# jzbontar/mc-cnn

Hardware: AMD Instinct MI355X
Metric: Mega-pixel-disparities/sec (cost-vol+CBCA+SGM) + end-to-end disp ms/pair (higher is better)
Workload: dtype f32; 1 GPU; KITTI 2012 fast, 370x1226 disp_max=228; H=370, W=1226, disp_max=228, feature_channels=64, params=kitti_fast, parallelism=one pair per GPU

## Files before the change

mc-cnn_amd/csrc/post.hip:

```cpp
#include "launchers.h"

#include <atomic>

namespace mc {


__global__ void __launch_bounds__(256) fill_nan_kernel(float *__restrict__ p, int64_t n)
{
	const float nanv = __builtin_nanf("");
	for (int64_t i = (int64_t)blockIdx.x * blockDim.x + threadIdx.x; i < n; i += (int64_t)gridDim.x * blockDim.x) p[i] = nanv;
}

__global__ void __launch_bounds__(256) scale_kernel(const float *__restrict__ in, float *__restrict__ out, int64_t n, float s)
{
	for (int64_t i = (int64_t)blockIdx.x * blockDim.x + threadIdx.x; i < n; i += (int64_t)gridDim.x * blockDim.x) out[i] = in[i] * s;
}
typedef float f4v_t __attribute__((ext_vector_type(4)));
__global__ void __launch_bounds__(256) scale4_kernel(const f4v_t *__restrict__ in, f4v_t *__restrict__ out, int64_t n4, float s)
{
	const int64_t i = (int64_t)blockIdx.x * 256 + threadIdx.x;
	if (i < n4) out[i] = in[i] * s;
}

template <bool NT>
__global__ void __launch_bounds__(256) transpose_kernel(const float *__restrict__ in, float *__restrict__ out, int64_t R,
                                                        int64_t Cn, int64_t ldin, int64_t ldout, float s)
{
	__shared__ float tile[64][65];
	const int64_t c0 = (int64_t)blockIdx.x * 64, r0 = (int64_t)blockIdx.y * 64;
	const int tx = threadIdx.x & 63, ty = threadIdx.x >> 6;
	for (int k = ty; k < 64; k += 4) {
		const int64_t r = r0 + k, c = c0 + tx;
		if (r < R && c < Cn) tile[k][tx] = NT ? __builtin_nontemporal_load(in + r * ldin + c) : in[r * ldin + c];
	}
	__syncthreads();
	for (int k = ty; k < 64; k += 4) {
		const int64_t c = c0 + k, r = r0 + tx;
		if (r < R && c < Cn) {
			if (NT) __builtin_nontemporal_store(tile[tx][k] * s, out + c * ldout + r);
			else out[c * ldout + r] = tile[tx][k] * s;
		}
	}
}

typedef float post_f4 __attribute__((ext_vector_type(4)));
template <bool NT, bool LOOP_R>
__global__ void __launch_bounds__(256) transpose4_kernel(const float *__restrict__ in, float *__restrict__ out, int64_t R,
                                                         int64_t Cn, int64_t ldin, int64_t ldout, float s)
{
	__shared__ float tile[64][65];
	const int lx = threadIdx.x & 15, ly = threadIdx.x >> 4;
	const int64_t fixed0 = (int64_t)blockIdx.x * 64;
	const int64_t nloop = LOOP_R ? R : Cn;
	for (int64_t t0 = 0; t0 < nloop; t0 += 64) {
		const int64_t c0 = LOOP_R ? fixed0 : t0, r0 = LOOP_R ? t0 : fixed0;
#pragma unroll
		for (int k = 0; k < 4; ++k) {
			const int row = ly + 16 * k;
			const int64_t r = r0 + row, c = c0 + 4 * lx;
			if (r < R && c < Cn) {
				const post_f4 *p = (const post_f4 *)(in + r * ldin + c);
				const post_f4 v = NT ? __builtin_nontemporal_load(p) : *p;
				tile[row][4 * lx + 0] = v.x; tile[row][4 * lx + 1] = v.y; tile[row][4 * lx + 2] = v.z; tile[row][4 * lx + 3] = v.w;
			}
		}
		__syncthreads();
#pragma unroll
		for (int k = 0; k < 4; ++k) {
			const int col = ly + 16 * k;
			const int64_t c = c0 + col, r = r0 + 4 * lx;
			if (c < Cn && r < R) {
				const post_f4 v = {tile[4 * lx + 0][col] * s, tile[4 * lx + 1][col] * s, tile[4 * lx + 2][col] * s, tile[4 * lx + 3][col] * s};
				post_f4 *q = (post_f4 *)(out + c * ldout + r);
				if (NT) __builtin_nontemporal_store(v, q);
				else *q = v;
			}
		}
		__syncthreads();
	}
}


int fill_nan(float *p, int64_t n, hipStream_t st)
{
	if (n <= 0) return 0;
	const unsigned blocks = cdiv(n, 256) < 4096u ? cdiv(n, 256) : 4096u;
	hipLaunchKernelGGL(fill_nan_kernel, dim3(blocks), dim3(256), 0, st, p, n);
	return check_launch("fill_nan");
}

int scale(const float *in, float *out, int64_t n, float s, hipStream_t st)
{
	if (n <= 0) return 0;
	if (n % 4 == 0 && (uintptr_t)in % 16 == 0 && (uintptr_t)out % 16 == 0 && n / 4 / 256 < 0x7fffffff) {
		hipLaunchKernelGGL(scale4_kernel, dim3(cdiv(n / 4, 256)), dim3(256), 0, st, (const f4v_t *)in, (f4v_t *)out, n / 4, s);
		return check_launch("scale");
	}
	const unsigned blocks = cdiv(n, 256) < 4096u ? cdiv(n, 256) : 4096u;
	hipLaunchKernelGGL(scale_kernel, dim3(blocks), dim3(256), 0, st, in, out, n, s);
	return check_launch("scale");
}

int transpose(const float *in, float *out, int64_t R, int64_t Cn, int64_t ldin, int64_t ldout, float s, hipStream_t st, int nt)
{
	const bool use_nt = nt >= 0 ? nt != 0 : R * Cn * 4 > ((int64_t)768 << 20);
	const bool aligned16 = Cn % 4 == 0 && ldin % 4 == 0 && ldout % 4 == 0 && (uintptr_t)in % 16 == 0 && (uintptr_t)out % 16 == 0;
	if (R % 4 == 0 && aligned16) {
		if (R <= Cn) {
			if (use_nt) hipLaunchKernelGGL((transpose4_kernel<true, true>), dim3(cdiv(Cn, 64)), dim3(256), 0, st, in, out, R, Cn, ldin, ldout, s);
			else hipLaunchKernelGGL((transpose4_kernel<false, true>), dim3(cdiv(Cn, 64)), dim3(256), 0, st, in, out, R, Cn, ldin, ldout, s);
		} else {
			if (use_nt) hipLaunchKernelGGL((transpose4_kernel<true, false>), dim3(cdiv(R, 64)), dim3(256), 0, st, in, out, R, Cn, ldin, ldout, s);
			else hipLaunchKernelGGL((transpose4_kernel<false, false>), dim3(cdiv(R, 64)), dim3(256), 0, st, in, out, R, Cn, ldin, ldout, s);
		}
		return check_launch("transpose");
	}
	if (use_nt) hipLaunchKernelGGL(transpose_kernel<true>, dim3(cdiv(Cn, 64), cdiv(R, 64)), dim3(256), 0, st, in, out, R, Cn, ldin, ldout, s);
	else hipLaunchKernelGGL(transpose_kernel<false>, dim3(cdiv(Cn, 64), cdiv(R, 64)), dim3(256), 0, st, in, out, R, Cn, ldin, ldout, s);
	return check_launch("transpose");
}

__global__ void __launch_bounds__(256) fix_border_kernel(float *__restrict__ vol, int64_t rows, int W, int n, int direction)
{
	const int64_t id = (int64_t)blockIdx.x * blockDim.x + threadIdx.x;
	if (id >= rows * n) return;
	const int i = (int)(id % n) + 1;
	const int64_t r = id / n;
	const int dst = direction < 0 ? W - i : i - 1;
	const int src = direction < 0 ? W - (n + 1) : n;
	vol[r * W + dst] = vol[r * W + src];
}

int fix_border(float *vol, int D, int H, int W, int n, int direction, hipStream_t st)
{
	if (n <= 0) return 0;
	const int64_t rows = (int64_t)D * H;
	hipLaunchKernelGGL(fix_border_kernel, dim3(cdiv(rows * n, 256)), dim3(256), 0, st, vol, rows, W, n, direction);
	return check_launch("fix_border");
}

__global__ void __launch_bounds__(256) argmin_dhw_kernel(const float *__restrict__ vol, float *__restrict__ out, int D, int64_t HW,
                                                         int base1)
{
	const int64_t p = (int64_t)blockIdx.x * blockDim.x + threadIdx.x;
	if (p >= HW) return;
	int argmin = 0;
	float mn = __builtin_inff();
	for (int i = 0; i < D; ++i) {
		const float val = __builtin_nontemporal_load(vol + i * HW + p);
		if (val < mn) {
			mn = val;
			argmin = i;
		}
	}
	out[p] = (float)(argmin + base1);
}

__global__ void __launch_bounds__(256) argmin_dhw4_kernel(const float *__restrict__ vol, float *__restrict__ out, int D, int64_t HW,
                                                          int base1)
{
	const int64_t p = ((int64_t)blockIdx.x * blockDim.x + threadIdx.x) * 4;
	if (p >= HW) return;
	int a0 = 0, a1 = 0, a2 = 0, a3 = 0;
	float m0 = __builtin_inff(), m1 = m0, m2 = m0, m3 = m0;
	for (int i = 0; i < D; ++i) {
		const post_f4 v = __builtin_nontemporal_load((const post_f4 *)(vol + i * HW + p));
		if (v.x < m0) { m0 = v.x; a0 = i; }
		if (v.y < m1) { m1 = v.y; a1 = i; }
		if (v.z < m2) { m2 = v.z; a2 = i; }
		if (v.w < m3) { m3 = v.w; a3 = i; }
	}
	*(post_f4 *)(out + p) = post_f4{(float)(a0 + base1), (float)(a1 + base1), (float)(a2 + base1), (float)(a3 + base1)};
}

int argmin_dhw(const float *vol, float *out, int D, int H, int W, int base1, hipStream_t st)
{
	const int64_t HW = (int64_t)H * W;
	if (HW % 4 == 0 && (uintptr_t)vol % 16 == 0 && (uintptr_t)out % 16 == 0)
		hipLaunchKernelGGL(argmin_dhw4_kernel, dim3(cdiv(HW / 4, 256)), dim3(256), 0, st, vol, out, D, HW, base1);
	else
		hipLaunchKernelGGL(argmin_dhw_kernel, dim3(cdiv(HW, 256)), dim3(256), 0, st, vol, out, D, HW, base1);
	return check_launch("argmin_dhw");
}

__global__ void __launch_bounds__(256) outlier_rows_kernel(const float *__restrict__ d0, const float *__restrict__ d1,
                                                           float *__restrict__ outlier, int W, int disp_max)
{
	extern __shared__ unsigned char mark[];
	const int y = blockIdx.x;
	const int64_t row = (int64_t)y * W;
	for (int x = threadIdx.x; x < W; x += 256) mark[x] = 0;
	__syncthreads();
	for (int xp = threadIdx.x; xp < W; xp += 256) {
		const float v = d1[row + xp];
		if (v > -2.0f && v < (float)disp_max + 2.0f) {
			const int base = (int)floorf(v);
#pragma unroll
			for (int k = -2; k <= 3; ++k) {
				const int d = base + k;
				if (d >= 0 && d < disp_max && xp + d < W && (double)fabsf((float)d - v) < 1.1) mark[xp + d] = 1;
			}
		}
	}
	__syncthreads();
	for (int x = threadIdx.x; x < W; x += 256) {
		const int64_t id = row + x;
		const int d0i = (int)d0[id];
		float res;
		if (x - d0i < 0) res = 1;
		else if ((double)fabsf(d0[id] - d1[id - d0i]) < 1.1) res = 0;
		else res = mark[x] ? 2.0f : 1.0f;
		outlier[id] = res;
	}
}

struct LdsRaised {
	std::atomic<int> cus[64] = {};
	int raise(const void *kernel, int bytes, const char *who, int *ncu = nullptr)
	{
		int dev = 0;
		hipError_t e = hipGetDevice(&dev);
		if (e == hipSuccess && (dev < 0 || dev >= 64)) e = hipErrorInvalidDevice;
		if (e != hipSuccess) {
			set_error("%s: hipGetDevice: %s (device %d)", who, hipGetErrorString(e), dev);
			return (int)e;
		}
		int n = cus[dev].load(std::memory_order_acquire);
		if (!n) {
			e = hipFuncSetAttribute(kernel, hipFuncAttributeMaxDynamicSharedMemorySize, bytes);
			if (e == hipSuccess) e = hipDeviceGetAttribute(&n, hipDeviceAttributeMultiprocessorCount, dev);
			if (e != hipSuccess || n <= 0) {
				set_error("%s: %d bytes of dynamic LDS on device %d: %s", who, bytes, dev, hipGetErrorString(e));
				return e != hipSuccess ? (int)e : MC_EINVAL;
			}
			cus[dev].store(n, std::memory_order_release);
		}
		if (ncu) *ncu = n;
		return 0;
	}
};

int outlier_detection(const float *d0, const float *d1, float *outlier, int H, int W, int disp_max, hipStream_t st)
{
	MC_REQUIRE(W <= 160 * 1024, "outlier_detection: a row of %d pixels needs more than the 160 KiB of LDS its marks live in", W);
	if (W > 64 * 1024) {
		static LdsRaised raised;
		const int rc = raised.raise((const void *)outlier_rows_kernel, 160 * 1024, "outlier_detection");
		if (rc) return rc;
	}
	hipLaunchKernelGGL(outlier_rows_kernel, dim3(H), dim3(256), (size_t)W, st, d0, d1, outlier, W, disp_max);
	return check_launch("outlier_detection");
}

__global__ void __launch_bounds__(256) interp_occ_rows_kernel(const float *__restrict__ d0, const float *__restrict__ outlier,
                                                              float *__restrict__ out, int W, unsigned *__restrict__ mask, int size)
{
	__shared__ int carry[256];
	__shared__ int first_valid;
	const int y = blockIdx.x, t = threadIdx.x;
	const int64_t row = (int64_t)y * W;
	if (mask) {
		const int wa = (int)((row + 31) >> 5), wb = (int)((row + W + 31) >> 5);
		for (int w0 = wa; w0 < wb; w0 += 8) {
			const int p = w0 * 32 + t;
			const uint64_t bal = __ballot(p < size && outlier[p] == 2);
			const int w = w0 + (t >> 5);
			if ((t & 31) == 0 && w < wb) mask[w] = (unsigned)(bal >> (t & 32));
		}
	}
	const int seg = (W + 255) / 256;
	const int xa = t * seg, xb = min(W, xa + seg);
	if (t == 0) first_valid = W;
	int last = -1;
	for (int x = xa; x < xb; ++x)
		if (outlier[row + x] == 0) last = x;
	carry[t] = last;
	__syncthreads();
	if (last >= 0) {
		int f = -1;
		for (int x = xa; x < xb; ++x)
			if (outlier[row + x] == 0) { f = x; break; }
		atomicMin(&first_valid, f);
	}
	for (int off = 1; off < 256; off <<= 1) {
		const int o = t >= off ? carry[t - off] : -1;
		__syncthreads();
		carry[t] = max(carry[t], o);
		__syncthreads();
	}
	int lv = t > 0 ? carry[t - 1] : -1;
	const int fv = first_valid;
	for (int x = xa; x < xb; ++x) {
		const int64_t id = row + x;
		const float o = outlier[id];
		if (o == 0) lv = x;
		float r = d0[id];
		if (o == 1) {
			if (lv >= 0) r = d0[row + lv];
			else if (fv < W) r = d0[row + fv];
		}
		out[id] = r;
	}
}

int interpolate_occlusion(const float *d0, const float *outlier, float *out, int H, int W, hipStream_t st, unsigned *mask)
{
	if (mask) MC_REQUIRE((int64_t)H * W < ((int64_t)1 << 31), "interpolate_occlusion: %dx%d pixels do not fit the mask's 32-bit index", H, W);
	hipLaunchKernelGGL(interp_occ_rows_kernel, dim3(H), dim3(256), 0, st, d0, outlier, out, W, mask, mask ? H * W : 0);
	return check_launch("interpolate_occlusion");
}

template <int K> __device__ __forceinline__ void ray_rank_step(float v, int inb, int &less, int &eq)
{
	const float ov = __uint_as_float(__builtin_amdgcn_update_dpp(0u, __float_as_uint(v), 0x120 + K, 0xf, 0xf, false));
	const int oin = __builtin_amdgcn_update_dpp(0, inb, 0x120 + K, 0xf, 0xf, false);
	less += (oin && ov < v) ? 1 : 0;
	eq += (oin && ov == v) ? 1 : 0;
}

#define MC_MIS_NU 4
constexpr int MIS_NT = 1024;
constexpr unsigned MIS_OOB = 0x80000000u;

__device__ __forceinline__ void ray_select(float v, int inb, int ray, int id, const float *__restrict__ d0, float *__restrict__ out)
{
	int less = 0, eq = inb;
	ray_rank_step<1>(v, inb, less, eq); ray_rank_step<2>(v, inb, less, eq); ray_rank_step<3>(v, inb, less, eq);
	ray_rank_step<4>(v, inb, less, eq); ray_rank_step<5>(v, inb, less, eq); ray_rank_step<6>(v, inb, less, eq);
	ray_rank_step<7>(v, inb, less, eq); ray_rank_step<8>(v, inb, less, eq); ray_rank_step<9>(v, inb, less, eq);
	ray_rank_step<10>(v, inb, less, eq); ray_rank_step<11>(v, inb, less, eq); ray_rank_step<12>(v, inb, less, eq);
	ray_rank_step<13>(v, inb, less, eq); ray_rank_step<14>(v, inb, less, eq); ray_rank_step<15>(v, inb, less, eq);
	const uint64_t bal = __ballot(inb != 0);
	const int n = __builtin_popcount((unsigned)((bal >> ((threadIdx.x & 48))) & 0xffffu));
	if (n == 0) {
		if (ray == 0) out[id] = d0[id];
		return;
	}
	const int want = n / 2;
	if (inb && less <= want && want < less + eq) out[id] = v;
}

__device__ __forceinline__ void mis_rays_masked(const float *__restrict__ d0, const float *__restrict__ outlier, float *__restrict__ out,
                                                int size, int H, int W, const unsigned *__restrict__ mask, int per)
{
	static_assert(MC_MIS_NU == 4, "the round below is two whole-pixel steps");
	extern __shared__ unsigned mis_lds[];
	__shared__ int wave_n[MIS_NT / 64];
	__shared__ int next_item;
	const int nw = (size + 31) >> 5;
	unsigned *lmask = mis_lds;
	unsigned *slot = lmask + nw;
	int *list_y = (int *)(slot + MIS_NT * 16);
	unsigned short *list = (unsigned short *)(list_y + MIS_NT);
	const int tid = threadIdx.x, lane = tid & 63, wid = tid >> 6;
	const int pa = blockIdx.x * per, pb = min(size, pa + per);
	if (pa >= pb) return;
	for (int i = tid; i < nw; i += MIS_NT) lmask[i] = mask[i];
	constexpr unsigned HX_LO = 0x10000012u, HX_HI = 0x34444432u, HY_LO = 0x00123444u, HY_HI = 0x44321000u;
	const unsigned xmax2 = 2u * (unsigned)W - 2u, ymax2 = 2u * (unsigned)H - 2u;
	for (int c0 = pa; c0 < pb; c0 += MIS_NT) {
		const int p = c0 + tid;
		bool mis = false;
		if (p < pb) {
			const float v = d0[p];
			mis = outlier[p] == 2;
			if (!mis) out[p] = v;
		}
		const uint64_t bal = __ballot(mis);
		if (lane == 0) wave_n[wid] = __builtin_popcountll(bal);
		if (tid == 0) next_item = MIS_NT;
		__syncthreads();
		int base = 0, nlist = 0;
#pragma unroll
		for (int k = 0; k < MIS_NT / 64; ++k) {
			const int c = wave_n[k];
			base += k < wid ? c : 0;
			nlist += c;
		}
		if (mis) {
			const int j = base + __builtin_popcountll(bal & (((uint64_t)1 << lane) - 1));
			list[j] = (unsigned short)tid;
			list_y[j] = p / W;
		}
		__syncthreads();
		const int nitems = nlist * 16;
		int i = tid;
		int q = 0, X2 = 0, Y2 = 0, sx = 0, sy = 0, o1 = 0, o2 = 0;
		auto start = [&]() {
			const int j = i >> 4, ray = i & 15, sh = 4 * (ray & 7);
			sx = (int)(((ray < 8 ? HX_LO : HX_HI) >> sh) & 15u) - 2;
			sy = (int)(((ray < 8 ? HY_LO : HY_HI) >> sh) & 15u) - 2;
			q = c0 + list[j];
			const int y = list_y[j];
			X2 = 2 * (q - y * W);
			Y2 = 2 * y;
			o1 = ((sy + 1) >> 1) * W + ((sx + 1) >> 1);
			o2 = sy * W + sx;
		};
		if (i < nitems) start();
		while (i < nitems) {
			const int o[MC_MIS_NU] = {o1, o2, o2 + o1, 2 * o2};
			unsigned off[MC_MIS_NU], m[MC_MIS_NU];
#pragma unroll
			for (int k = 0; k < MC_MIS_NU; ++k) {
				X2 += sx;
				Y2 += sy;
				const bool in = (unsigned)X2 <= xmax2 && (unsigned)Y2 <= ymax2;
				const unsigned a = in ? (unsigned)(q + o[k]) : 0u;
				off[k] = in ? a : MIS_OOB;
				m[k] = lmask[a >> 5] >> (a & 31);
				m[k] = in ? m[k] & 1u : 0u;
			}
			q += 2 * o2;
			unsigned stop = MIS_OOB;
			bool stopped = false;
#pragma unroll
			for (int k = MC_MIS_NU - 1; k >= 0; --k) {
				const bool hit = m[k] == 0;
				stop = hit ? off[k] : stop;
				stopped = hit ? true : stopped;
			}
			if (stopped) {
				slot[i] = stop;
				i = atomicAdd(&next_item, 1);
				if (i < nitems) start();
			}
		}
		__syncthreads();
		const int ray = tid & 15;
		int j = tid >> 4;
		unsigned stop = j < nlist ? slot[j * 16 + ray] : MIS_OOB;
		float v = d0[stop != MIS_OOB ? stop : 0u];
		while (j < nlist) {
			const int jn = j + MIS_NT / 16;
			const unsigned stop_n = jn < nlist ? slot[jn * 16 + ray] : MIS_OOB;
			const float v_n = d0[stop_n != MIS_OOB ? stop_n : 0u];
			ray_select(stop != MIS_OOB ? v : 0.0f, stop != MIS_OOB ? 1 : 0, ray, c0 + list[j], d0, out);
			j = jn;
			stop = stop_n;
			v = v_n;
		}
		__syncthreads();
	}
}

__global__ void __launch_bounds__(MIS_NT) interp_mis_rays_kernel(const float *__restrict__ d0, const float *__restrict__ outlier,
                                                                 float *__restrict__ out, int size, int H, int W,
                                                                 const unsigned *__restrict__ mask, int per)
{
	if (mask) {
		mis_rays_masked(d0, outlier, out, size, H, W, mask, per);
		return;
	}
	const int t = blockIdx.x * blockDim.x + threadIdx.x;
	const int id = t >> 4;
	const int ray = (int)(threadIdx.x & 15);
	if (id >= size) return;
	const bool mis = outlier[id] == 2;
	if (!mis) {
		if (ray == 0) out[id] = d0[id];
		return;
	}
	const int hx[16] = {0, -1, -2, -2, -2, -2, -2, -1, 0, 1, 2, 2, 2, 2, 2, 1};
	const int hy[16] = {2, 2, 2, 1, 0, -1, -2, -2, -2, -2, -2, -1, 0, 1, 2, 2};
	const int x = id % W, y = id / W;
	const int sx = hx[ray], sy = hy[ray];
	const __amdgpu_buffer_rsrc_t ro = __builtin_amdgcn_make_buffer_rsrc((void *)outlier, 0, size * 4, 0x00020000);
	const __amdgpu_buffer_rsrc_t rd = __builtin_amdgcn_make_buffer_rsrc((void *)d0, 0, size * 4, 0x00020000);
	int X2 = 2 * x, Y2 = 2 * y;
	constexpr unsigned OOB = MIS_OOB;
	unsigned stop = OOB;
	for (bool go = true; go;) {
		unsigned off[MC_MIS_NU], o[MC_MIS_NU];
#pragma unroll
		for (int i = 0; i < MC_MIS_NU; ++i) {
			X2 += sx;
			Y2 += sy;
			const int xi = (X2 + 1 + (X2 >> 31)) >> 1;
			const int yi = (Y2 + 1 + (Y2 >> 31)) >> 1;
			const bool in = (unsigned)yi < (unsigned)H && (unsigned)xi < (unsigned)W;
			off[i] = in ? (__umul24((unsigned)yi, (unsigned)W) + (unsigned)xi) * 4u : OOB;
			o[i] = __builtin_amdgcn_raw_buffer_load_b32(ro, off[i], 0, 0);
		}
#pragma unroll
		for (int i = MC_MIS_NU - 1; i >= 0; --i) {
			const bool hit = __uint_as_float(o[i]) != 2.0f;
			stop = hit ? off[i] : stop;
			go = hit ? false : go;
		}
	}
	const int inb = stop != OOB ? 1 : 0;
	const float v = __uint_as_float(__builtin_amdgcn_raw_buffer_load_b32(rd, stop, 0, 0));
	ray_select(v, inb, ray, id, d0, out);
}

int interpolate_mismatch(const float *d0, const float *outlier, float *out, int H, int W, hipStream_t st, const unsigned *mask)
{
	const int64_t size = (int64_t)H * W;
	MC_REQUIRE(size * 16 < ((int64_t)1 << 31), "interpolate_mismatch: %dx%d pixels x 16 rays do not fit a 32-bit index", H, W);
	MC_REQUIRE(H < (1 << 24) && W < (1 << 24), "interpolate_mismatch: %dx%d: a side beyond the 24-bit row / column arithmetic of the ray walk", H, W);
	if (mask && size <= MC_MIS_MASK_MAX_PIXELS) {
		constexpr int MAX_LDS = MC_MIS_MASK_MAX_PIXELS / 8 + MIS_NT * (16 * 4 + 4 + 2);
		static LdsRaised raised;
		int cus = 0;
		const int rc = raised.raise((const void *)interp_mis_rays_kernel, MAX_LDS, "interpolate_mismatch", &cus);
		if (rc) return rc;
		const int blocks = (int)min((int64_t)cus, (int64_t)cdiv(size, MIS_NT));
		const int per = (int)(cdiv(size, blocks) + 63) / 64 * 64;
		const size_t lds = (size_t)((size + 31) / 32) * 4 + MIS_NT * (16 * 4 + 4 + 2);
		hipLaunchKernelGGL(interp_mis_rays_kernel, dim3(blocks), dim3(MIS_NT), lds, st, d0, outlier, out, (int)size, H, W, mask, per);
		return check_launch("interpolate_mismatch");
	}
	hipLaunchKernelGGL(interp_mis_rays_kernel, dim3(cdiv(size * 16, 256)), dim3(256), 0, st, d0, outlier, out, (int)size, H, W,
	                   (const unsigned *)nullptr, 0);
	return check_launch("interpolate_mismatch");
}

__global__ void __launch_bounds__(256) subpixel_kernel(const float *__restrict__ d0, const float *__restrict__ c2,
                                                       float *__restrict__ out, int64_t size, int64_t sd, int64_t sp, int disp_max,
                                                       float *__restrict__ cost_out, float *__restrict__ curv_out)
{
	const int64_t id = (int64_t)blockIdx.x * blockDim.x + threadIdx.x;
	if (id >= size) return;
	const int d = (int)d0[id];
	float res = (float)d;
	if (1 <= d && d < disp_max - 1) {
		const float cn = c2[(d - 1) * sd + id * sp];
		const float cz = c2[d * sd + id * sp];
		const float cp = c2[(d + 1) * sd + id * sp];
		const float denom = 2 * (cp + cn - 2 * cz);
		if ((double)denom > 1e-5) {
			res = (float)((double)d - fmin(1.0, fmax(-1.0, (double)((cp - cn) / denom))));
		}
		if (cost_out) cost_out[id] = cz;
		if (curv_out) curv_out[id] = denom;
	} else {
		if (cost_out) cost_out[id] = (0 <= d && d < disp_max) ? c2[d * sd + id * sp] : __int_as_float(0x7fc00000);
		if (curv_out) curv_out[id] = 0;
	}
	out[id] = res;
}

int subpixel_conf(const float *d0, const float *vol, float *out, int D, int H, int W, int64_t sd, int64_t sp, hipStream_t st, float *cost_out,
                  float *curv_out)
{
	const int64_t size = (int64_t)H * W;
	hipLaunchKernelGGL(subpixel_kernel, dim3(cdiv(size, 256)), dim3(256), 0, st, d0, vol, out, size, sd, sp, D, cost_out, curv_out);
	return check_launch("subpixel_enchancement");
}

int subpixel(const float *d0, const float *vol, float *out, int D, int H, int W, int64_t sd, int64_t sp, hipStream_t st)
{
	return subpixel_conf(d0, vol, out, D, H, W, sd, sp, st, nullptr, nullptr);
}

__device__ __forceinline__ void cswap(float &a, float &b)
{
	const float lo = fminf(a, b), hi = fmaxf(a, b);
	a = lo;
	b = hi;
}

template <int N>
__device__ __forceinline__ float median_forgetful(const float (&v)[N])
{
	constexpr int M0 = N / 2 + 2;
	float w[M0];
#pragma unroll
	for (int i = 0; i < M0; ++i) w[i] = v[i];
	int next = M0;
#pragma unroll
	for (int m = M0; m > 3; --m) {
#pragma unroll
		for (int i = 0; i < m / 2; ++i) cswap(w[i], w[m - 1 - i]);
#pragma unroll
		for (int i = 1; i < (m + 1) / 2; ++i) cswap(w[0], w[i]);
#pragma unroll
		for (int i = m / 2; i < m - 1; ++i) cswap(w[i], w[m - 1]);
		w[0] = v[next < N ? next : N - 1];
		++next;
	}
	cswap(w[0], w[1]);
	cswap(w[1], w[2]);
	cswap(w[0], w[1]);
	return w[1];
}

template <int KR>
__global__ void __launch_bounds__(256) median_kernel(const float *__restrict__ img, float *__restrict__ out, int H, int W)
{
	constexpr int K = 2 * KR + 1;
	constexpr int TW = 64 + 2 * KR, TH = 4 + 2 * KR;
	__shared__ float tile[TH][TW + 1];
	const int bx = blockIdx.x * 64, by = blockIdx.y * 4;
	for (int i = threadIdx.x; i < TH * TW; i += 256) {
		const int ty = i / TW, tx = i % TW;
		const int gx = bx + tx - KR, gy = by + ty - KR;
		tile[ty][tx] = (gx >= 0 && gx < W && gy >= 0 && gy < H) ? img[(int64_t)gy * W + gx] : 0.0f;
	}
	__syncthreads();
	const int lx = threadIdx.x & 63, ly = threadIdx.x >> 6;
	const int x = bx + lx, y = by + ly;
	if (x >= W || y >= H) return;
	const int xa = max(0, x - KR), xb = min(W - 1, x + KR), ya = max(0, y - KR), yb = min(H - 1, y + KR);
	const int n = (xb - xa + 1) * (yb - ya + 1);
	if constexpr (KR == 1 || KR == 2) {
		float v[K * K];
#pragma unroll
		for (int i = 0; i < K * K; ++i) v[i] = tile[ly + i % K][lx + i / K];
		if (n != K * K) {
			int lo = K * K / 2 - n / 2;
#pragma unroll
			for (int i = 0; i < K * K; ++i) {
				const int ix = x - KR + i / K, iy = y - KR + i % K;
				if (ix < xa || ix > xb || iy < ya || iy > yb) v[i] = lo-- > 0 ? -__builtin_inff() : __builtin_inff();
			}
		}
		out[(int64_t)y * W + x] = median_forgetful<K * K>(v);
		return;
	}
	const int want = n / 2;
	float res = 0;
	for (int i = 0; i < K * K; ++i) {
		const int ix = x - KR + i / K, iy = y - KR + i % K;
		if (ix < xa || ix > xb || iy < ya || iy > yb) continue;
		const float vi = tile[iy - by + KR][ix - bx + KR];
		int less = 0, eq = 0;
		for (int yy = ya; yy <= yb; ++yy) {
			for (int xx = xa; xx <= xb; ++xx) {
				const float vj = tile[yy - by + KR][xx - bx + KR];
				less += vj < vi ? 1 : 0;
				eq += vj == vi ? 1 : 0;
			}
		}
		if (less <= want && want < less + eq) {
			res = vi;
			break;
		}
	}
	out[(int64_t)y * W + x] = res;
}

int median2d(const float *img, float *out, int H, int W, int k, hipStream_t st)
{
	const dim3 grid(cdiv(W, 64), cdiv(H, 4)), block(256);
	switch (k / 2) {
	case 0: hipLaunchKernelGGL(median_kernel<0>, grid, block, 0, st, img, out, H, W); break;
	case 1: hipLaunchKernelGGL(median_kernel<1>, grid, block, 0, st, img, out, H, W); break;
	case 2: hipLaunchKernelGGL(median_kernel<2>, grid, block, 0, st, img, out, H, W); break;
	case 3: hipLaunchKernelGGL(median_kernel<3>, grid, block, 0, st, img, out, H, W); break;
	case 4: hipLaunchKernelGGL(median_kernel<4>, grid, block, 0, st, img, out, H, W); break;
	default: hipLaunchKernelGGL(median_kernel<5>, grid, block, 0, st, img, out, H, W); break;
	}
	return check_launch("median2d");
}

constexpr int M2_OY = 2;
constexpr int M2_TR = 4;
__global__ void __launch_bounds__(64 * M2_TR) mean2d_kernel(const float *__restrict__ img, const float *__restrict__ kernel,
                                                            float *__restrict__ out, int H, int W, int kr, float alpha2)
{
	extern __shared__ __attribute__((aligned(16))) float smem[];
	constexpr int NT = 64 * M2_TR;
	const int ks = 2 * kr + 1;
	const int TW = 64 + 2 * kr, TH = M2_TR * M2_OY + 2 * kr;
	const int TS = TW + 1;
	const int WS = ks + 2 * (M2_OY - 1);
	float *tile = smem;
	float *wts = smem + TH * TS;
	const int bx = blockIdx.x * 64, by = blockIdx.y * (M2_TR * M2_OY);
	const float FAR = 1e30f;
	for (int i = threadIdx.x; i < TH * TW; i += NT) {
		const int ty = i / TW, tx = i - ty * TW;
		const int gx = bx + tx - kr, gy = by + ty - kr;
		tile[ty * TS + tx] = (gx >= 0 && gx < W && gy >= 0 && gy < H) ? img[(int64_t)gy * W + gx] : FAR;
	}
	for (int i = threadIdx.x; i < ks * WS; i += NT) {
		const int ix = i / WS, j = i - ix * WS - (M2_OY - 1);
		wts[i] = (j >= 0 && j < ks) ? kernel[ix * ks + j] : -0.0f;
	}
	__syncthreads();
	const int lx = threadIdx.x & 63, ly = threadIdx.x >> 6;
	const int x = bx + lx, yb = by + ly * M2_OY;
	if (x >= W || yb >= H) return;
	float c[M2_OY], sum[M2_OY], cnt[M2_OY];
#pragma unroll
	for (int o = 0; o < M2_OY; ++o) {
		c[o] = tile[(ly * M2_OY + o + kr) * TS + lx + kr];
		sum[o] = 0.0f;
		cnt[o] = 0.0f;
	}
	const int nj = ks + M2_OY - 1;
	for (int ix = 0; ix < ks; ++ix) {
		const float *col = tile + (ly * M2_OY) * TS + lx + ix;
		const float *wc = wts + ix * WS + (M2_OY - 1);
		float wprev[M2_OY > 1 ? M2_OY - 1 : 1];
#pragma unroll
		for (int o = 0; o < M2_OY - 1; ++o) wprev[o] = -0.0f;
#pragma unroll 4
		for (int j = 0; j < nj; ++j) {
			const float v = col[0];
			col += TS;
			const float w0 = wc[j];
			float ws[M2_OY];
			ws[0] = w0;
#pragma unroll
			for (int o = 1; o < M2_OY; ++o) ws[o] = wprev[o - 1];
#pragma unroll
			for (int o = 0; o < M2_OY; ++o) {
				const float w = fabsf(v - c[o]) < alpha2 ? ws[o] : -0.0f;
				sum[o] = fmaf(v, w, sum[o]);
				cnt[o] += w;
			}
#pragma unroll
			for (int o = M2_OY - 2; o > 0; --o) wprev[o] = wprev[o - 1];
			if (M2_OY > 1) wprev[0] = w0;
		}
	}
#pragma unroll
	for (int o = 0; o < M2_OY; ++o)
		if (yb + o < H) out[(int64_t)(yb + o) * W + x] = sum[o] / cnt[o];
}

#define MC_M2_TAP(i) \
	"v_sub_f32 %[d], %[v" #i "], %[c]\n\tv_cmpx_lt_f32_e64 vcc, |%[d]|, %[a]\n\tv_fmac_f32 %[s], %[w" #i "], %[v" #i "]\n\t" \
	"v_add_f32 %[n], %[w" #i "], %[n]\n\ts_mov_b64 exec, %[e]\n\t"
__device__ __forceinline__ void mean2d_taps8(float &sum, float &cnt, const float (&v)[8], const float (&w)[8], float c, float alpha2,
                                             unsigned long long ex)
{
	float d;
	asm volatile(MC_M2_TAP(0) MC_M2_TAP(1) MC_M2_TAP(2) MC_M2_TAP(3) MC_M2_TAP(4) MC_M2_TAP(5) MC_M2_TAP(6) MC_M2_TAP(7)
	             : [s] "+v"(sum), [n] "+v"(cnt), [d] "=&v"(d)
	             : [v0] "v"(v[0]), [v1] "v"(v[1]), [v2] "v"(v[2]), [v3] "v"(v[3]), [v4] "v"(v[4]), [v5] "v"(v[5]), [v6] "v"(v[6]),
	               [v7] "v"(v[7]), [w0] "s"(w[0]), [w1] "s"(w[1]), [w2] "s"(w[2]), [w3] "s"(w[3]), [w4] "s"(w[4]), [w5] "s"(w[5]),
	               [w6] "s"(w[6]), [w7] "s"(w[7]), [c] "v"(c), [a] "s"(alpha2), [e] "s"(ex)
	             : "vcc");
}
__device__ __forceinline__ void mean2d_tap1(float &sum, float &cnt, float v0, float w0, float c, float alpha2, unsigned long long ex)
{
	float d;
	asm volatile(MC_M2_TAP(0) : [s] "+v"(sum), [n] "+v"(cnt), [d] "=&v"(d)
	             : [v0] "v"(v0), [w0] "s"(w0), [c] "v"(c), [a] "s"(alpha2), [e] "s"(ex)
	             : "vcc");
}
#undef MC_M2_TAP

template <int KR>
__global__ void __launch_bounds__(512) mean2d_taps_kernel(const float *__restrict__ img, const float *__restrict__ kernel,
                                                          float *__restrict__ out, int H, int W, float alpha2)
{
	constexpr int KS = 2 * KR + 1, TW = 64 + 2 * KR, TH = 8 + 2 * KR, TS = TW + 1;
	__shared__ float tile[TH * TS];
	const int bx = blockIdx.x * 64, by = blockIdx.y * 8;
	const float FAR = 1e30f;
	for (int i = threadIdx.x; i < TH * TW; i += 512) {
		const int ty = i / TW, tx = i - ty * TW;
		const int gx = bx + tx - KR, gy = by + ty - KR;
		tile[ty * TS + tx] = (gx >= 0 && gx < W && gy >= 0 && gy < H) ? img[(int64_t)gy * W + gx] : FAR;
	}
	__syncthreads();
	const int lx = threadIdx.x & 63, ly = threadIdx.x >> 6;
	const int x = bx + lx, y = by + ly;
	if (x >= W || y >= H) return;
	const unsigned long long ex = __builtin_amdgcn_read_exec();
	const float c = tile[(ly + KR) * TS + lx + KR];
	float sum = 0.0f, cnt = 0.0f;
	const float *col = tile + ly * TS + lx;
	for (int ix = 0; ix < KS; ++ix, ++col) {
		const float *wc = kernel + ix * KS;
#pragma unroll
		for (int j0 = 0; j0 + 8 <= KS; j0 += 8) {
			float v[8], w[8];
#pragma unroll
			for (int g = 0; g < 8; ++g) {
				v[g] = col[(j0 + g) * TS];
				w[g] = wc[j0 + g];
			}
			__builtin_amdgcn_sched_barrier(0);
			mean2d_taps8(sum, cnt, v, w, c, alpha2, ex);
			__builtin_amdgcn_sched_barrier(0);
		}
#pragma unroll
		for (int j = KS / 8 * 8; j < KS; ++j) mean2d_tap1(sum, cnt, col[j * TS], wc[j], c, alpha2, ex);
	}
	out[(int64_t)y * W + x] = sum / cnt;
}

template <int KR>
static int mean2d_taps(const float *img, const float *kernel, float *out, int H, int W, float alpha2, hipStream_t st)
{
	hipLaunchKernelGGL(mean2d_taps_kernel<KR>, dim3(cdiv(W, 64), cdiv(H, 8)), dim3(512), 0, st, img, kernel, out, H, W, alpha2);
	return check_launch("mean2d");
}

int mean2d(const float *img, const float *kernel, float *out, int H, int W, int ks, float alpha2, hipStream_t st)
{
	switch (ks) {
	case 13: return mean2d_taps<6>(img, kernel, out, H, W, alpha2, st);
	case 19: return mean2d_taps<9>(img, kernel, out, H, W, alpha2, st);
	case 29: return mean2d_taps<14>(img, kernel, out, H, W, alpha2, st);
	case 37: return mean2d_taps<18>(img, kernel, out, H, W, alpha2, st);
	case 49: return mean2d_taps<24>(img, kernel, out, H, W, alpha2, st);
	default: break;
	}
	const int kr = ks / 2;
	const size_t lds =
	    ((size_t)(M2_TR * M2_OY + 2 * kr) * (64 + 2 * kr + 1) + (size_t)ks * (ks + 2 * (M2_OY - 1))) * sizeof(float);
	if (lds > 160 * 1024) {
		set_error("mean2d: kernel size %d needs %zu B of LDS (> 160 KiB)", ks, lds);
		return MC_EINVAL;
	}
	if (lds > 64 * 1024) {
		hipError_t e = hipFuncSetAttribute((const void *)mean2d_kernel, hipFuncAttributeMaxDynamicSharedMemorySize, (int)lds);
		if (e != hipSuccess) {
			set_error("mean2d: hipFuncSetAttribute: %s", hipGetErrorString(e));
			return (int)e;
		}
	}
	hipLaunchKernelGGL(mean2d_kernel, dim3(cdiv(W, 64), cdiv(H, M2_TR * M2_OY)), dim3(64 * M2_TR), lds, st, img, kernel, out, H, W, kr,
	                   alpha2);
	return check_launch("mean2d");
}

template <int CT>
__global__ void __launch_bounds__(256) normalize_kernel(const float *__restrict__ in, float *__restrict__ norm, float *__restrict__ out,
                                                        int C, int64_t HW, int64_t NHW)
{
	const int64_t id = (int64_t)blockIdx.x * blockDim.x + threadIdx.x;
	if (id >= NHW) return;
	const int64_t n = id / HW, p = id % HW;
	const float *src = in + n * C * HW + p;
	float *dst = out + n * C * HW + p;
	float sum = 0.0f;
	if constexpr (CT > 0) {
		float v[CT];
#pragma unroll
		for (int c = 0; c < CT; ++c) v[c] = c < C ? __builtin_nontemporal_load(src + c * HW) : 0.0f;
#pragma unroll
		for (int c = 0; c < CT; ++c)
			if (c < C) sum = fmaf(v[c], v[c], sum);
		const float nv = (float)((double)sum + 1e-5);
		if (norm) norm[id] = nv;
		const float r = sqrtf(nv);
#pragma unroll
		for (int c = 0; c < CT; ++c)
			if (c < C) dst[c * HW] = v[c] / r;
	} else {
		for (int c = 0; c < C; ++c) {
			const float x = src[c * HW];
			sum = fmaf(x, x, sum);
		}
		const float nv = (float)((double)sum + 1e-5);
		if (norm) norm[id] = nv;
		const float r = sqrtf(nv);
		for (int c = 0; c < C; ++c) dst[c * HW] = src[c * HW] / r;
	}
}

int normalize_forward(const float *in, float *norm, float *out, int N, int C, int H, int W, hipStream_t st)
{
	const int64_t HW = (int64_t)H * W;
	const dim3 grid(cdiv(N * HW, 256)), block(256);
	if (C <= 64) hipLaunchKernelGGL(normalize_kernel<64>, grid, block, 0, st, in, norm, out, C, HW, N * HW);
	else if (C <= 128) hipLaunchKernelGGL(normalize_kernel<128>, grid, block, 0, st, in, norm, out, C, HW, N * HW);
	else hipLaunchKernelGGL(normalize_kernel<0>, grid, block, 0, st, in, norm, out, C, HW, N * HW);
	return check_launch("normalize_forward");
}

}
```

mc-cnn_amd/csrc/sgm.hip:

```cpp
#include "sgm_line.h"

#include <atomic>

namespace mc {

__device__ __forceinline__ int cls_of(float v, float tau) { return v < tau ? 0 : (v > tau ? 2 : 1); }

__global__ void __launch_bounds__(256) sgm_prep_kernel(const float *__restrict__ x0, const float *__restrict__ x1,
                                                       uint8_t *__restrict__ cls0, uint8_t *__restrict__ win,
                                                       int H, int W, int Wm, int64_t cls_plane, float tau_so)
{
	const int64_t id = (int64_t)blockIdx.x * blockDim.x + threadIdx.x;
	const int64_t total = (int64_t)4 * H * Wm;
	if (id >= total) return;
	const int i = (int)(id % Wm);
	const int y = (int)((id / Wm) % H);
	const int r = (int)(id / ((int64_t)Wm * H));
	const int dx = r == 0 ? 1 : (r == 1 ? -1 : 0);
	const int dy = r == 2 ? 1 : (r == 3 ? -1 : 0);
	const bool yok = (y - dy >= 0) && (y - dy < H);

	if (i < W) {
		const int x = i;
		int c = 1;
		if (yok && x - dx >= 0 && x - dx < W) {
			c = cls_of(fabsf(x0[y * W + x] - x0[(y - dy) * W + x - dx]), tau_so);
		}
		cls0[(int64_t)r * cls_plane + (int64_t)y * W + x] = (uint8_t)c;
	}
	const int s = i - ((Wm - W) >> 1);
	unsigned asc = 0, desc = 0;
#pragma unroll
	for (int k = 0; k < 4; ++k) {
		const int xx = s + k;
		float D2 = 10.0f;
		if (yok && xx >= 0 && xx < W && xx - dx >= 0 && xx - dx < W) {
			D2 = fabsf(x1[y * W + xx] - x1[(y - dy) * W + xx - dx]);
		}
		const unsigned c = (unsigned)cls_of(D2, tau_so);
		asc |= c << (2 * k);
		desc |= c << (2 * (3 - k));
	}
	win[((int64_t)(0 * 4 + r) * H + y) * Wm + i] = (uint8_t)asc;
	win[((int64_t)(1 * 4 + r) * H + y) * Wm + i] = (uint8_t)desc;
}


__global__ void __launch_bounds__(256) sgm_contract_kernel(const float *__restrict__ vol, int64_t pixels, int D, unsigned *__restrict__ count)
{
	const int64_t p = (int64_t)blockIdx.x * blockDim.x + threadIdx.x;
	bool bad = false;
	if (p < pixels) {
		const float *v = vol + p * D;
		bad = !(fabsf(v[0]) < __builtin_inff());
		bool seen_nan = false;
		for (int d = 0; d < D; ++d) {
			const bool isn = v[d] != v[d];
			bad = bad || (seen_nan && !isn);
			seen_nan = seen_nan || isn;
		}
	}
	const unsigned long long b = __ballot(bad);
	if ((threadIdx.x & 63) == 0 && b) atomicAdd(count, (unsigned)__builtin_popcountll(b));
}

int sgm_contract_violations(const float *vol, int H, int W, int D, unsigned *count, hipStream_t st)
{
	const int64_t pixels = (int64_t)H * W;
	hipError_t e = hipMemsetAsync(count, 0, sizeof(unsigned), st);
	if (e != hipSuccess) {
		set_error("mc_sgm2_contract_violations: hipMemsetAsync: %s", hipGetErrorString(e));
		return (int)e;
	}
	hipLaunchKernelGGL(sgm_contract_kernel, dim3(cdiv(pixels, 256)), dim3(256), 0, st, vol, pixels, D, count);
	return check_launch("sgm_contract");
}

struct SgmMaps { int Wm; size_t plane, cls0, win, bytes; };
static SgmMaps sgm_maps(int H, int W, int D)
{
	const int Wm = W + 2 * sgm_padw(D);
	const size_t plane = ((size_t)H * W + 3 + 4) / 4 * 4;
	return {Wm, plane, 0, 4 * plane, (4 * plane + (size_t)8 * H * Wm + 255) & ~(size_t)255};
}

size_t sgm_maps_bytes(int H, int W) { return sgm_maps(H, W, 1).bytes; }
size_t sgm_maps_bytes_d(int H, int W, int D) { return sgm_maps(H, W, D).bytes; }

int sgm_prep(const float *x0, const float *x1, void *maps, int H, int W, float tau_so, hipStream_t st)
{
	return sgm_prep_d(x0, x1, maps, H, W, 1, tau_so, st);
}

int sgm_prep_d(const float *x0, const float *x1, void *maps, int H, int W, int D, float tau_so, hipStream_t st)
{
	const SgmMaps m = sgm_maps(H, W, D);
	const int64_t total = (int64_t)4 * H * m.Wm;
	hipLaunchKernelGGL(sgm_prep_kernel, dim3(cdiv(total, 256)), dim3(256), 0, st, x0, x1, (uint8_t *)maps + m.cls0, (uint8_t *)maps + m.win, H, W,
	                   m.Wm, (int64_t)m.plane, tau_so);
	return check_launch("sgm_prep");
}

constexpr int SGM_U_H = 8, SGM_U_UP = 16;
constexpr int SGM_U_DOWN = 16;

template <int DIRN, int MODE, bool ARGMIN, bool DUAL>
static void launch_pass(const SgmPassArgs &A, bool vec, hipStream_t st)
{
	const int nlines = DIRN <= 1 ? A.H : A.W;
	const int waves = A.nvol * nlines * (DUAL ? 2 : 1);
	const dim3 grid(cdiv(waves, 4)), block(256);
	const int U = DIRN == 2 ? SGM_U_DOWN : (DIRN == 3 ? SGM_U_UP : SGM_U_H);
	constexpr bool SCALAR = MODE == 1;
#define MC_SGM_GO(VPL_, VEC_, U_) \
	hipLaunchKernelGGL((sgm_pass_kernel<DIRN, VPL_, MODE, ARGMIN, VEC_, U_, DUAL, false>), grid, block, 0, st, A)
#define MC_SGM_GO_FAR(VPL_, VEC_, U_) \
	hipLaunchKernelGGL((sgm_pass_kernel<DIRN, VPL_, MODE, ARGMIN, VEC_, U_, DUAL, true>), grid, block, 0, st, A)
	const bool far = sgm_far(A.H, A.W, A.ds);
	if (A.D > 512) {
		MC_SGM_GO(8, true, 8);
	} else if (!vec) {
		if constexpr (SCALAR) {
			if (far) { if (A.D <= 256) MC_SGM_GO_FAR(4, false, 4); else MC_SGM_GO_FAR(8, false, 2); }
			else { if (A.D <= 256) MC_SGM_GO(4, false, 4); else MC_SGM_GO(8, false, 2); }
		}
	} else if (far) {
		if (A.D <= 256) MC_SGM_GO_FAR(4, true, 4); else MC_SGM_GO_FAR(8, true, 4);
	} else if (A.D <= 256) {
		if (U == 16) MC_SGM_GO(4, true, 16); else if (U == 8) MC_SGM_GO(4, true, 8); else MC_SGM_GO(4, true, 4);
	} else {
		if (U >= 8) MC_SGM_GO(8, true, 8); else MC_SGM_GO(8, true, 4);
	}
#undef MC_SGM_GO_FAR
#undef MC_SGM_GO
}


int sgm_vertical(int set)
{
	static std::atomic<int> forced{0};
	if (set >= 0 && set <= 2) forced.store(set);
	const int f = forced.load();
	return f ? f : 2;
}

int sgm_sweeps(const float *const C[2], float *const out[2], float *const out2[2], float *const disp[2],
               const int direction[2], int nvol, int H, int W, int D, int ds, const void *maps, float pi1, float pi2,
               float alpha1, float q1, float q2, bool fused, unsigned drop_final, bool tri, hipStream_t st)
{
	return sgm_sweeps_ck(C, out, out2, disp, direction, nvol, H, W, D, ds, maps, pi1, pi2, alpha1, q1, q2, fused, drop_final, tri, nullptr, st);
}

int sgm_sweeps_ck(const float *const C[2], float *const out[2], float *const out2[2], float *const disp[2],
                  const int direction[2], int nvol, int H, int W, int D, int ds, const void *maps, float pi1, float pi2,
                  float alpha1, float q1, float q2, bool fused, unsigned drop_final, bool tri, float *const ck[2], hipStream_t st)
{
	MC_REQUIRE((int64_t)H * W < ((int64_t)1 << 29) && (int64_t)W * ds * 4 < ((int64_t)1 << 31), "sgm: image %dx%d (pixel stride %d) exceeds the sweeps' 32-bit line arithmetic", H, W, ds);
	SgmPassArgs A;
	for (int v = 0; v < 2; ++v) {
		const int k = v < nvol ? v : 0;
		A.C[v] = C[k];
		A.accin[v] = out[k];
		A.accin2[v] = out2 ? out2[k] : nullptr;
		A.out[v] = out[k];
		A.out2[v] = out2 ? out2[k] : nullptr;
		A.disp[v] = disp ? disp[k] : nullptr;
		A.direction[v] = direction[k];
		A.drop_out[v] = 0;
		A.drop_h[v] = (fused && tri && v < nvol && ((drop_final >> v) & 1)) ? 1 : 0;
		A.ck[v] = ck ? ck[k] : nullptr;
	}
	A.nvol = nvol;
	A.tri = (fused && tri) ? 1 : 0;
	A.H = H; A.W = W; A.D = D; A.ds = ds;
	const SgmMaps m = sgm_maps(H, W, D);
	A.Wm = m.Wm;
	A.cls0 = (const uint8_t *)maps + m.cls0;
	A.cls_plane = (int64_t)m.plane;
	A.win = (const uint8_t *)maps + m.win;
	A.P1[0] = pi1; A.P2[0] = pi2;
	A.P1[1] = pi1 / q1; A.P2[1] = pi2 / q1;
	A.P1[2] = pi1 / (q1 * q2); A.P2[2] = pi2 / (q1 * q2);
	for (int k = 0; k < 3; ++k) A.P1a[k] = A.P1[k] / alpha1;

	const bool vec = sgm_vec(A);
	const bool am = fused && disp && disp[0];
	if (!fused) {
		launch_pass<0, 1, false, false>(A, vec, st);
		launch_pass<1, 1, false, false>(A, vec, st);
		launch_pass<2, 1, false, false>(A, vec, st);
		launch_pass<3, 1, false, false>(A, vec, st);
	} else {
		MC_REQUIRE(out2 && vec, "sgm: the fused sweeps need the second direction's scratch and 16-byte aligned volumes with ds %% 4 == 0");
		launch_pass<0, 0, false, true>(A, vec, st);
		if (const int rc = check_launch("sgm_pass horizontal")) return rc;
		const bool far = sgm_far(H, W, ds);
		bool slots = ck != nullptr;
		for (int v = 0; v < nvol && slots; ++v) slots = ck[v] && (uintptr_t)ck[v] % 16 == 0;
		if (slots && D <= 256 && !far && sgm_vertical() == 2) {
			MC_REQUIRE(mc_sgm_recompute_launch(&A, sizeof A, 0, st) == 0, "sgm: the checkpoint launch was refused");
			if (const int rc = check_launch("sgm_pass down checkpoints")) return rc;
			for (int v = 0; v < nvol; ++v) A.drop_out[v] = (drop_final >> v) & 1;
			MC_REQUIRE(mc_sgm_recompute_launch(&A, sizeof A, am ? 2 : 1, st) == 0, "sgm: the recomputing launch was refused");
			return check_launch("sgm_pass up, down recomputed");
		}
		launch_pass<2, 3, false, false>(A, vec, st);
		if (const int rc = check_launch("sgm_pass down")) return rc;
		for (int v = 0; v < nvol; ++v) A.drop_out[v] = (drop_final >> v) & 1;
		if (am) launch_pass<3, 2, true, false>(A, vec, st);
		else launch_pass<3, 2, false, false>(A, vec, st);
		return check_launch("sgm_pass up");
	}
	return check_launch("sgm_pass");
}

}
```

Before: 96100 MPix-disp/s.

## Transpose mean2d tile for float4 LDS reads; vectorize SGM prep byte writes

```diff
diff --git a/mc-cnn_amd/csrc/post.hip b/mc-cnn_amd/csrc/post.hip
--- a/mc-cnn_amd/csrc/post.hip
+++ b/mc-cnn_amd/csrc/post.hip
@@ -746,42 +746,74 @@
 #undef MC_M2_TAP
 
 template <int KR>
+constexpr int m2_row_stride()
+{
+	const int r = (8 + 2 * KR + 3) / 4 * 4;
+	return (r / 4) % 2 ? r : r + 4;
+}
+
+template <int KR, int O, int G0>
+__device__ __forceinline__ void mean2d_tap_groups(const float *__restrict__ col, const float *__restrict__ wc, float c, float alpha2,
+                                                  unsigned long long ex, float &sum, float &cnt)
+{
+	constexpr int KS = 2 * KR + 1, NG = (O + KS + 3) / 4;
+	if constexpr (G0 < NG) {
+		constexpr int jlo = 4 * G0 - O;
+		const float4 q0 = *(const float4 *)(col + 4 * G0);
+		const float4 q1 = *(const float4 *)(col + 4 * (G0 + 1 < NG ? G0 + 1 : G0));
+		const float v[8] = {q0.x, q0.y, q0.z, q0.w, q1.x, q1.y, q1.z, q1.w};
+		float w[8];
+#pragma unroll
+		for (int e = 0; e < 8; ++e) w[e] = (jlo + e >= 0 && jlo + e < KS) ? wc[jlo + e] : 0.0f;
+		__builtin_amdgcn_sched_barrier(0);
+		if constexpr (jlo >= 0 && jlo + 8 <= KS) {
+			mean2d_taps8(sum, cnt, v, w, c, alpha2, ex);
+		} else {
+#pragma unroll
+			for (int e = 0; e < 8; ++e)
+				if (jlo + e >= 0 && jlo + e < KS) mean2d_tap1(sum, cnt, v[e], w[e], c, alpha2, ex);
+		}
+		__builtin_amdgcn_sched_barrier(0);
+		mean2d_tap_groups<KR, O, G0 + 2>(col, wc, c, alpha2, ex, sum, cnt);
+	}
+}
+
+template <int KR, int O>
+__device__ __forceinline__ void mean2d_tap_columns(const float *__restrict__ colbase, const float *__restrict__ kernel, float c, float alpha2,
+                                                   unsigned long long ex, float &sum, float &cnt)
+{
+	constexpr int KS = 2 * KR + 1, RS = m2_row_stride<KR>();
+	const float *col = colbase;
+	for (int ix = 0; ix < KS; ++ix, col += RS) mean2d_tap_groups<KR, O, 0>(col, kernel + ix * KS, c, alpha2, ex, sum, cnt);
+}
+
+template <int KR>
 __global__ void __launch_bounds__(512) mean2d_taps_kernel(const float *__restrict__ img, const float *__restrict__ kernel,
                                                           float *__restrict__ out, int H, int W, float alpha2)
 {
-	constexpr int KS = 2 * KR + 1, TW = 64 + 2 * KR, TH = 8 + 2 * KR, TS = TW + 1;
-	__shared__ float tile[TH * TS];
+	constexpr int TW = 64 + 2 * KR, TH = 8 + 2 * KR, RS = m2_row_stride<KR>();
+	static_assert(RS % 4 == 0 && (RS / 4) % 2 == 1 && RS >= TH, "mean2d: the transposed tile's row stride");
+	__shared__ __attribute__((aligned(16))) float tileT[TW * RS];
 	const int bx = blockIdx.x * 64, by = blockIdx.y * 8;
 	const float FAR = 1e30f;
 	for (int i = threadIdx.x; i < TH * TW; i += 512) {
 		const int ty = i / TW, tx = i - ty * TW;
 		const int gx = bx + tx - KR, gy = by + ty - KR;
-		tile[ty * TS + tx] = (gx >= 0 && gx < W && gy >= 0 && gy < H) ? img[(int64_t)gy * W + gx] : FAR;
+		tileT[tx * RS + ty] = (gx >= 0 && gx < W && gy >= 0 && gy < H) ? img[(int64_t)gy * W + gx] : FAR;
 	}
 	__syncthreads();
-	const int lx = threadIdx.x & 63, ly = threadIdx.x >> 6;
+	const int lx = threadIdx.x & 63, ly = __builtin_amdgcn_readfirstlane(threadIdx.x >> 6);
 	const int x = bx + lx, y = by + ly;
 	if (x >= W || y >= H) return;
 	const unsigned long long ex = __builtin_amdgcn_read_exec();
-	const float c = tile[(ly + KR) * TS + lx + KR];
+	const float c = tileT[(lx + KR) * RS + ly + KR];
 	float sum = 0.0f, cnt = 0.0f;
-	const float *col = tile + ly * TS + lx;
-	for (int ix = 0; ix < KS; ++ix, ++col) {
-		const float *wc = kernel + ix * KS;
-#pragma unroll
-		for (int j0 = 0; j0 + 8 <= KS; j0 += 8) {
-			float v[8], w[8];
-#pragma unroll
-			for (int g = 0; g < 8; ++g) {
-				v[g] = col[(j0 + g) * TS];
-				w[g] = wc[j0 + g];
-			}
-			__builtin_amdgcn_sched_barrier(0);
-			mean2d_taps8(sum, cnt, v, w, c, alpha2, ex);
-			__builtin_amdgcn_sched_barrier(0);
-		}
-#pragma unroll
-		for (int j = KS / 8 * 8; j < KS; ++j) mean2d_tap1(sum, cnt, col[j * TS], wc[j], c, alpha2, ex);
+	const float *colbase = tileT + lx * RS + (ly & ~3);
+	switch (ly & 3) {
+	case 0: mean2d_tap_columns<KR, 0>(colbase, kernel, c, alpha2, ex, sum, cnt); break;
+	case 1: mean2d_tap_columns<KR, 1>(colbase, kernel, c, alpha2, ex, sum, cnt); break;
+	case 2: mean2d_tap_columns<KR, 2>(colbase, kernel, c, alpha2, ex, sum, cnt); break;
+	default: mean2d_tap_columns<KR, 3>(colbase, kernel, c, alpha2, ex, sum, cnt); break;
 	}
 	out[(int64_t)y * W + x] = sum / cnt;
 }
diff --git a/mc-cnn_amd/csrc/sgm.hip b/mc-cnn_amd/csrc/sgm.hip
--- a/mc-cnn_amd/csrc/sgm.hip
+++ b/mc-cnn_amd/csrc/sgm.hip
@@ -10,39 +10,101 @@
                                                        uint8_t *__restrict__ cls0, uint8_t *__restrict__ win,
                                                        int H, int W, int Wm, int64_t cls_plane, float tau_so)
 {
-	const int64_t id = (int64_t)blockIdx.x * blockDim.x + threadIdx.x;
-	const int64_t total = (int64_t)4 * H * Wm;
-	if (id >= total) return;
-	const int i = (int)(id % Wm);
-	const int y = (int)((id / Wm) % H);
-	const int r = (int)(id / ((int64_t)Wm * H));
-	const int dx = r == 0 ? 1 : (r == 1 ? -1 : 0);
-	const int dy = r == 2 ? 1 : (r == 3 ? -1 : 0);
-	const bool yok = (y - dy >= 0) && (y - dy < H);
-
-	if (i < W) {
-		const int x = i;
-		int c = 1;
-		if (yok && x - dx >= 0 && x - dx < W) {
-			c = cls_of(fabsf(x0[y * W + x] - x0[(y - dy) * W + x - dx]), tau_so);
-		}
-		cls0[(int64_t)r * cls_plane + (int64_t)y * W + x] = (uint8_t)c;
-	}
-	const int s = i - ((Wm - W) >> 1);
-	unsigned asc = 0, desc = 0;
-#pragma unroll
-	for (int k = 0; k < 4; ++k) {
-		const int xx = s + k;
+	using I = int64_t;
+	const I t = (I)blockIdx.x * blockDim.x + threadIdx.x;
+	const I HWm = (I)H * Wm;
+	if (t >= HWm) return;
+	const bool words = (((uintptr_t)cls0 | (uintptr_t)win) & 3) == 0;
+	const int pad = (Wm - W) >> 1;
+	const unsigned cfar = (unsigned)cls_of(10.0f, tau_so) * 0x55u;
+	auto dx_of = [](int r) { return r == 0 ? 1 : (r == 1 ? -1 : 0); };
+	auto dy_of = [](int r) { return r == 2 ? 1 : (r == 3 ? -1 : 0); };
+
+	auto cls1 = [&](int y, int xx, int dx, int dy, bool yok) -> unsigned {
 		float D2 = 10.0f;
 		if (yok && xx >= 0 && xx < W && xx - dx >= 0 && xx - dx < W) {
 			D2 = fabsf(x1[y * W + xx] - x1[(y - dy) * W + xx - dx]);
 		}
-		const unsigned c = (unsigned)cls_of(D2, tau_so);
-		asc |= c << (2 * k);
-		desc |= c << (2 * (3 - k));
-	}
-	win[((int64_t)(0 * 4 + r) * H + y) * Wm + i] = (uint8_t)asc;
-	win[((int64_t)(1 * 4 + r) * H + y) * Wm + i] = (uint8_t)desc;
+		return (unsigned)cls_of(D2, tau_so);
+	};
+	unsigned asc4 = 0, desc4 = 0;
+	{
+		const I id = 4 * t;
+		const I row = id / (I)Wm;
+		const int i = (int)(id - row * (I)Wm);
+		if (i + 3 < Wm) {
+			const int r = (int)(row / (I)H), y = (int)(row - (I)r * (I)H);
+			const int dx = dx_of(r), dy = dy_of(r);
+			const bool yok = (y - dy >= 0) && (y - dy < H);
+			const int s = i - pad;
+			if (!yok || s + 6 < 0 || s >= W) {
+				asc4 = desc4 = cfar * 0x01010101u;
+			} else {
+				unsigned c[7];
+#pragma unroll
+				for (int k = 0; k < 7; ++k) c[k] = cls1(y, s + k, dx, dy, yok);
+#pragma unroll
+				for (int b = 0; b < 4; ++b) {
+					asc4 |= (c[b] | c[b + 1] << 2 | c[b + 2] << 4 | c[b + 3] << 6) << (8 * b);
+					desc4 |= (c[b] << 6 | c[b + 1] << 4 | c[b + 2] << 2 | c[b + 3]) << (8 * b);
+				}
+			}
+		} else {
+			for (int b = 0; b < 4; ++b) {
+				const bool next = i + b >= Wm;
+				const int ib = next ? i + b - Wm : i + b;
+				const I rowb = next ? row + 1 : row;
+				const int r = (int)(rowb / (I)H), y = (int)(rowb - (I)r * (I)H);
+				const int dx = dx_of(r), dy = dy_of(r);
+				const bool yok = (y - dy >= 0) && (y - dy < H);
+				const int s = ib - pad;
+				unsigned asc = 0, desc = 0;
+#pragma unroll
+				for (int k = 0; k < 4; ++k) {
+					const unsigned c = cls1(y, s + k, dx, dy, yok);
+					asc |= c << (2 * k);
+					desc |= c << (2 * (3 - k));
+				}
+				asc4 |= asc << (8 * b);
+				desc4 |= desc << (8 * b);
+			}
+		}
+		uint8_t *wa = win + (int64_t)id, *wd = win + 4 * (int64_t)HWm + (int64_t)id;
+		if (words) {
+			*(uint32_t *)wa = asc4;
+			*(uint32_t *)wd = desc4;
+		} else {
+			for (int b = 0; b < 4; ++b) {
+				wa[b] = (uint8_t)(asc4 >> (8 * b));
+				wd[b] = (uint8_t)(desc4 >> (8 * b));
+			}
+		}
+	}
+
+	if (t >= cls_plane) return;
+	const I pw = cls_plane >> 2;
+	const int r = (int)(t / pw);
+	const I p0 = (t - (I)r * pw) * 4;
+	const I HW = (I)H * (I)W;
+	if (p0 >= HW) return;
+	const int dx = dx_of(r), dy = dy_of(r);
+	unsigned c4 = 0;
+	int y = (int)(p0 / (I)W), x = (int)(p0 - (I)y * (I)W);
+#pragma unroll
+	for (int b = 0; b < 4; ++b) {
+		unsigned c = 1;
+		if (p0 + b < HW && (y - dy >= 0) && (y - dy < H) && x - dx >= 0 && x - dx < W) {
+			c = (unsigned)cls_of(fabsf(x0[y * W + x] - x0[(y - dy) * W + x - dx]), tau_so);
+		}
+		c4 |= c << (8 * b);
+		if (++x == W) { x = 0; ++y; }
+	}
+	uint8_t *cp = cls0 + (int64_t)r * (int64_t)cls_plane + (int64_t)p0;
+	if (words && p0 + 3 < HW) {
+		*(uint32_t *)cp = c4;
+	} else {
+		for (int b = 0; b < 4 && p0 + b < HW; ++b) cp[b] = (uint8_t)(c4 >> (8 * b));
+	}
 }
 
 
@@ -95,7 +157,8 @@
 int sgm_prep_d(const float *x0, const float *x1, void *maps, int H, int W, int D, float tau_so, hipStream_t st)
 {
 	const SgmMaps m = sgm_maps(H, W, D);
-	const int64_t total = (int64_t)4 * H * m.Wm;
+	MC_REQUIRE(m.plane % 4 == 0 && m.cls0 % 4 == 0 && m.win % 4 == 0, "sgm_prep: class planes of %zu bytes", m.plane);
+	const int64_t total = (int64_t)H * m.Wm;
 	hipLaunchKernelGGL(sgm_prep_kernel, dim3(cdiv(total, 256)), dim3(256), 0, st, x0, x1, (uint8_t *)maps + m.cls0, (uint8_t *)maps + m.win, H, W,
 	                   m.Wm, (int64_t)m.plane, tau_so);
 	return check_launch("sgm_prep");
```

Measured after the change: 96550 MPix-disp/s, median of 6. About the same (+0.5%).
